# givemeone1astkiss/RNA-MPNN

Measured on AMD Instinct MI355X. Metric: nucleotides/sec (forward), k=30 RNA graphs, higher is better.
Workload: dtype bf16; 1 GPU; C2: batch=256 RNAs, n~U[100,140], k=30, default 10-layer RNAMPNN, P=T; max_len=140, weights=closed-form deterministic init (3,536,900 params), parallelism=dp1

## Files before the change

rna-mpnn_amd/csrc/api.cpp:

```cpp
#include "api_internal.h"
#include "kernels_bf16.h"

#include <cstdarg>
#include <cstdlib>
#include <cstdio>
#include <cstring>
#include <string>
#include <vector>

static thread_local char g_err[512] = "";

int fail(int code, const char* fmt, ...) {
    va_list ap;
    va_start(ap, fmt);
    vsnprintf(g_err, sizeof(g_err), fmt, ap);
    va_end(ap);
    return code;
}

extern "C" const char* rnampnn_last_error(void) { return g_err; }
extern "C" const char* rnampnn_version(void) { return "rnampnn-hip 0.1 (gfx950)"; }

static int add_raw(rnampnn_ctx* c, const std::string& key, int64_t numel) {
    RawT t{key, numel, c->raw_floats, false};
// ... 459 lines not shown
}

static void run_ffn(Run& r, const Chain& ch, const std::vector<Lin>& ffn, const float* x, int ldx, float* out) {
    if (run_chain(r, ch, ffn, x, ldx, nullptr, 0, out, ffn.back().out)) return;
    const float* cur = x;
    int ld = ldx;
    float* bufs[2] = {r.w.s0, r.w.s1};
    for (size_t i = 0; i < ffn.size(); ++i) {
        bool last = i + 1 == ffn.size();
        float* dst = last ? out : bufs[i & 1];
        gemm(r, ffn[i], cur, ld, dst, ffn[i].out);
        cur = dst; ld = ffn[i].out;
    }
}

static NodeJob node_job(rnampnn_ctx* c, const Mlp2& m, bf16_t* p, bf16_t* q) {
    NodeJob j;
    j.img = derp<bf16_t>(c, m.pq_img); j.bias = derp<float>(c, m.pq_bp); j.p = p; j.q = q; j.p_efrag = m.depth == 1;
    return j;
}
static void node_pq(Run& r, const Mlp2& m, const float* h, bool edge) {
    rnampnn_ctx* c = r.c;
    if (r.fast)
        launch_node_update(r.pk, h, nullptr, nullptr, 0, nullptr, nullptr, 1,
                           node_job(c, m, edge ? r.w.p_e : r.w.p_m, edge ? r.w.q_e : r.w.q_m), NodeJob{}, r.s);
    else
        launch_gemm_f32(r.ntot(), r.pk.Nmax, h, RN_D, RN_D, nullptr, 0, 0, derp<float>(c, m.pq_t),
                        derp<float>(c, m.pq_b), 256, 0, nullptr, 0, edge ? r.w.pq_e : r.w.pq_m, 256, r.s);
}

static MpnnW32 w32(rnampnn_ctx* c, const Mlp2& m) {
    MpnnW32 w;
    w.wc_t = derp<float>(c, m.wc_t);
    w.w2_t = m.depth > 1 ? derp<float>(c, m.w2_t) : nullptr;
    w.b2 = m.depth > 1 ? rawp(c, m.b[1]) : nullptr;
    w.depth = m.depth;
    return w;
}
static MpnnWB wbf(rnampnn_ctx* c, const Mlp2& m) {
    MpnnWB w;
    w.img = derp<bf16_t>(c, m.img);
    w.b2p = derp<float>(c, m.b2p);
    return w;
}

static void mpnn_step(Run& r, const Mlp2* we, const Mlp2* wm, const float* h_in, float* h_pre, float* msg_out, bool embed_first = false,
                      int reverse = 0) {
    rnampnn_ctx* c = r.c;
    int k = c->cfg.num_res_neighbours;
    bool timed = c->prof && c->ev_used + 2 <= c->ev.size() && (c->prof_seen++ % c->prof_stride) == 0;
    if (timed) { c->ev_kind[c->ev_used / 2] = (we && wm) ? 0 : 1; (void)hipEventRecord(c->ev[c->ev_used], r.s); }
    if (embed_first) {
        launch_resmpnn_embed_bf16(r.pk, k, r.w.nbr, (bf16_t*)r.w.e, r.w.geomh, derp<bf16_t>(c, c->edge_embed_img), rawp(c, c->edge_embed[0].b),
                                  derp<float>(c, c->edge_embed_b1p), r.w.p_m, r.w.q_m, wbf(c, *wm), h_pre, h_in, reverse, r.s);
    } else if (r.fast) {
        launch_mpnn_bf16(r.pk, k, we != nullptr, wm != nullptr, r.w.nbr, (bf16_t*)r.w.e, r.w.p_e, r.w.q_e, r.w.p_m,
                         r.w.q_m, we ? wbf(c, *we) : MpnnWB{}, wm ? wbf(c, *wm) : MpnnWB{}, h_pre, msg_out, we && we->depth == 1,
                         wm ? h_in : nullptr, reverse, r.s);
    } else {
        MpnnW32 e32 = we ? w32(c, *we) : MpnnW32{}, m32 = wm ? w32(c, *wm) : MpnnW32{};
        launch_mpnn_f32(r.pk, k, we != nullptr, wm != nullptr, r.w.nbr, (float*)r.w.e, r.w.pq_e, r.w.pq_m, e32, m32,
                        h_in, h_pre, msg_out, r.s);
    }
    if (timed) { (void)hipEventRecord(c->ev[c->ev_used + 1], r.s); c->ev_used += 2; }
}

static void unpack_e(Run& r, float* dst) {
    int k = r.c->cfg.num_res_neighbours;
    if (r.fast) {
        launch_efrag_to_rows((const bf16_t*)r.w.e, r.ntot(), r.pk.Nmax, k, r.w.big, r.s);
        launch_unpack_edges(r.pk, k, r.w.big, r.w.nbr, dst, r.s);
    } else {
        launch_unpack_edges(r.pk, k, (const float*)r.w.e, r.w.nbr, dst, r.s);
    }
}

static int begin_run(Run& r, rnampnn_handle h, const float* mask, int B, int T, void* ws, size_t ws_bytes, void* stream,
                     const int32_t* cu_seqlens = nullptr, int n_total = 0) {
    if (!h) return fail(RNAMPNN_ERR_BAD_ARG, "null handle");
    if (!h->finalized) return fail(RNAMPNN_ERR_WEIGHTS, "weights not finalized (call rnampnn_finalize_weights)");
    if ((!mask && !cu_seqlens) || !ws || B <= 0 || T <= 0) return fail(RNAMPNN_ERR_BAD_ARG, "null pointer or non-positive B/T");
    const long long nmax = cu_seqlens ? (long long)n_total : (long long)B * T;
    if (nmax <= 0 || nmax > 0x3fffffffLL / (h->cfg.num_res_neighbours * 4))
        return fail(RNAMPNN_ERR_BAD_ARG, "row count out of range for 32-bit edge indexing; split the batch");
    size_t need = carve(h, B, (size_t)nmax, nullptr, nullptr);
    if (ws_bytes < need) return fail(RNAMPNN_ERR_WORKSPACE, "workspace %zu bytes < required %zu", ws_bytes, need);
    if (((uintptr_t)ws & 255) != 0) return fail(RNAMPNN_ERR_BAD_ARG, "workspace must be 256-byte aligned");
    r.c = h;
    r.s = (hipStream_t)stream;
    r.fast = h->cfg.precision == RNAMPNN_PREC_BF16;
    carve(h, B, (size_t)nmax, (char*)ws, &r.w);
    r.pk.len = r.w.len; r.pk.cu = r.w.cu; r.pk.node_b = r.w.node_b;
    r.pk.B = B; r.pk.T = T; r.pk.Nmax = (int)nmax; r.pk.packed_in = cu_seqlens ? 1 : 0;
    size_t Nmax = r.pk.Nmax;
    ZeroRegions z{};
    auto add = [&](void* p, size_t bytes) { z.ptr[z.n] = p; z.words[z.n] = (unsigned)(bytes / 4); ++z.n; };
    add(r.w.hA + Nmax * RN_D, RN_D * sizeof(float));
    add(r.w.hB + Nmax * RN_D, RN_D * sizeof(float));
    if (r.fast) {
        add(r.w.p_e + Nmax * RN_D, RN_D * sizeof(bf16_t));
        add(r.w.p_m + Nmax * RN_D, RN_D * sizeof(bf16_t));
        add(r.w.q_e + Nmax * RN_D, RN_D * sizeof(bf16_t));
        add(r.w.q_m + Nmax * RN_D, RN_D * sizeof(bf16_t));
    } else {
        add(r.w.pq_e + Nmax * 256, 256 * sizeof(float));
        add(r.w.pq_m + Nmax * 256, 256 * sizeof(float));
    }
    if (cu_seqlens) launch_lengths_from_cu(cu_seqlens, r.pk, r.s);
    else launch_lengths(mask, r.pk, r.s);
    launch_zero_regions(z, r.s);
    return RNAMPNN_OK;
}

struct PackedOut { float* logits; float* embedding; int n_total; };
static int forward_core(Run& r, rnampnn_handle h, const RnaMpnnForwardIO* io, const PackedOut* po);

extern "C" int rnampnn_forward(rnampnn_handle h, const RnaMpnnForwardIO* io, void* ws, size_t ws_bytes, void* stream) {
    if (!io || !io->coords) return fail(RNAMPNN_ERR_BAD_ARG, "rnampnn_forward: null io/coords");
    if (io->stop_after == 0 && !io->logits && !io->embedding)
        return fail(RNAMPNN_ERR_BAD_ARG, "rnampnn_forward: logits (or embedding) output required");
    Run r;
    int rc = begin_run(r, h, io->mask, io->B, io->T, ws, ws_bytes, stream);
    if (rc) return rc;
    return forward_core(r, h, io, nullptr);
}

extern "C" int rnampnn_forward_packed(rnampnn_handle h, const float* coords_packed, const int32_t* cu_seqlens, int32_t B,
                                      int32_t N_total, int32_t T_max, int32_t T_norm, float* logits_packed,
                                      float* embedding_packed, void* ws, size_t ws_bytes, void* stream) {
    if (!coords_packed || !cu_seqlens || (!logits_packed && !embedding_packed))
        return fail(RNAMPNN_ERR_BAD_ARG, "rnampnn_forward_packed: null input or no output");
    Run r;
    int rc = begin_run(r, h, nullptr, B, T_max, ws, ws_bytes, stream, cu_seqlens, N_total);
    if (rc) return rc;
    RnaMpnnForwardIO io;
    memset(&io, 0, sizeof(io));
    io.coords = coords_packed; io.B = B; io.T = T_max; io.T_norm = T_norm;
    PackedOut po{logits_packed, embedding_packed, N_total};
    return forward_core(r, h, &io, &po);
}

static int forward_core(Run& r, rnampnn_handle h, const RnaMpnnForwardIO* io, const PackedOut* po) {
    int rc = RNAMPNN_OK;
    rnampnn_ctx* c = h;
    const RnaMpnnConfig& g = c->cfg;
    if (io->T > g.padding_len)
        return fail(RNAMPNN_ERR_T_GT_P, "max_len %d exceeds padding_len %d", io->T, g.padding_len);
    int k = g.num_res_neighbours, L = g.num_res_mpnn_layers;
    int t_norm = io->T_norm > 0 ? io->T_norm : io->T;
    if (t_norm < io->T) return fail(RNAMPNN_ERR_BAD_ARG, "T_norm %d < T %d", t_norm, io->T);
    Ws& w = r.w;
    hipStream_t s = r.s;

    launch_geom(io->coords, r.pk, t_norm, io->raw, w.raw_p, w.geom, r.fast ? w.geomh : nullptr, s);
    const bool fused_first = r.fast && io->stop_after != 1;
    {
        const Lin& l = c->raw_project;
        launch_gemm_f32(r.ntot(), r.pk.Nmax, w.raw_p, RN_RAWP, l.in_pad, nullptr, 0, 0, derp<float>(c, l.wt), rawp(c, l.b), l.out,
                        l.gelu ? 1 : 0, nullptr, 0, w.n0, RN_D, r.s);
    }
    rc = run_bert(r, c->emb, w.n0, w.n1);
    if (!rc) {
        if (fused_first)
            launch_node_update(r.pk, w.n1, rawp(c, c->feat_gn_scale), rawp(c, c->feat_gn_shift), t_norm, w.coef, w.hA, 1,
                               node_job(c, c->mpnn[0].msg, w.p_m, w.q_m), NodeJob{}, r.s);
        else
            launch_graph_norm_packed(r.pk, w.n1, w.hA, rawp(c, c->feat_gn_scale), rawp(c, c->feat_gn_shift), t_norm, r.s);
    }
    if (rc) return rc;
    if (launch_knn(io->coords, r.pk, t_norm, k, w.nbr, io->edge_index, s))
        return fail(RNAMPNN_ERR_UNSUPPORTED, "max_len %d too long for the LDS-resident k-NN row", io->T);
    const bool embed_first = fused_first && L >= 1 && !io->e0 && resmpnn_covers(k, false, false) && !ab_switch("RNAMPNN_EMBED_TWO_LAUNCH");
    if (embed_first) { }
    else if (r.fast)
        launch_edge_embed_bf16(r.pk, k, w.geomh, w.nbr, derp<bf16_t>(c, c->edge_embed_img), rawp(c, c->edge_embed[0].b),
                               derp<float>(c, c->edge_embed_b1p), (bf16_t*)w.e, s);
    else
        launch_edge_embed_f32(r.pk, k, w.geom, w.nbr, derp<float>(c, c->edge_embed[0].wt), rawp(c, c->edge_embed[0].b),
                              g.depth_res_edge_feature > 1 ? derp<float>(c, c->edge_embed[1].wt) : nullptr,
                              g.depth_res_edge_feature > 1 ? rawp(c, c->edge_embed[1].b) : nullptr,
                              g.depth_res_edge_feature, (float*)w.e, s);
    if (io->h0) launch_unpack_nodes(r.pk, w.hA, RN_D, RN_D, io->h0, s);
    if (io->e0) unpack_e(r, io->e0);
    if (io->stop_after == 1) { HIP_TRY(hipGetLastError()); return RNAMPNN_OK; }

    if (!fused_first) node_pq(r, c->mpnn[0].msg, w.hA, false);
    bool edge_pending = false;
    int n_fused = 0;
    for (int l = 0; l < L; ++l) {
        mpnn_step(r, edge_pending ? &c->mpnn[l - 1].edge : nullptr, &c->mpnn[l].msg, w.hA, w.hB, nullptr, l == 0 && embed_first, n_fused++ & 1);
        bool tap_e = io->tap_layer == l + 1 && io->e_layer;
        edge_pending = l + 1 < L;
        const bool need_e = edge_pending || tap_e, need_m = l + 1 < L;
        const float* gsc = rawp(c, c->mpnn[l].gn_scale);
        const float* gsh = rawp(c, c->mpnn[l].gn_shift);
        if (r.fast && (need_e || need_m)) {
            const NodeJob je = need_e ? node_job(c, c->mpnn[l].edge, w.p_e, w.q_e) : NodeJob{};
            const NodeJob jm = need_m ? node_job(c, c->mpnn[l + 1].msg, w.p_m, w.q_m) : NodeJob{};
            launch_node_update(r.pk, w.hB, gsc, gsh, t_norm, w.coef, w.hA, (need_e && need_m) ? 2 : 1, need_e ? je : jm, jm, s);
        } else {
            launch_graph_norm_packed(r.pk, w.hB, w.hA, gsc, gsh, t_norm, s);
            if (need_e) node_pq(r, c->mpnn[l].edge, w.hA, true);
            if (need_m) node_pq(r, c->mpnn[l + 1].msg, w.hA, false);
        }
        if (io->tap_layer == l + 1) {
            if (io->h_layer) launch_unpack_nodes(r.pk, w.hA, RN_D, RN_D, io->h_layer, s);
            if (tap_e) {
                mpnn_step(r, &c->mpnn[l].edge, nullptr, w.hA, w.hB, nullptr, false, n_fused++ & 1);
                edge_pending = false;
                unpack_e(r, io->e_layer);
            }
        }
    }
    float* raw_emb = w.n2;
    rc = run_bert(r, c->post, w.hA, w.n0);
    if (rc) return rc;
    run_ffn(r, c->raw_chain, c->raw_ffn, w.raw_p, RN_RAWP, w.n1);
    launch_graph_norm_packed(r.pk, w.n1, w.n2, rawp(c, c->rawffn_gn_scale), rawp(c, c->rawffn_gn_shift), t_norm, s);
    if (io->h_post) launch_unpack_nodes(r.pk, w.n0, RN_D, RN_D, io->h_post, s);
    if (io->raw_emb) launch_unpack_nodes(r.pk, raw_emb, RN_D, RN_D, io->raw_emb, s);
    if (io->embedding) {
        launch_unpack_nodes_strided(r.pk, w.n0, RN_D, RN_D, io->embedding, 2 * RN_D, 0, s);
        launch_unpack_nodes_strided(r.pk, raw_emb, RN_D, RN_D, io->embedding, 2 * RN_D, RN_D, s);
    }
    if (po && po->embedding) {
        HIP_TRY(hipMemcpy2DAsync(po->embedding, 2 * RN_D * sizeof(float), w.n0, RN_D * sizeof(float), RN_D * sizeof(float),
                                 po->n_total, hipMemcpyDeviceToDevice, s));
        HIP_TRY(hipMemcpy2DAsync(po->embedding + RN_D, 2 * RN_D * sizeof(float), raw_emb, RN_D * sizeof(float),
                                 RN_D * sizeof(float), po->n_total, hipMemcpyDeviceToDevice, s));
    }
    const bool want_logits = io->logits || (po && po->logits);
    float* logits_rows = (po && po->logits) ? po->logits : w.logits_p;
    if (want_logits && run_chain(r, c->readout_chain, c->readout, w.n0, RN_D, raw_emb, RN_D, logits_rows, 4)) {
        if (io->logits) launch_unpack_nodes(r.pk, logits_rows, 4, 4, io->logits, s);
    } else if (want_logits) {
        const float* cur = nullptr;
        int ld = 0;
        float* bufs[2] = {w.s0, w.s1};
        for (size_t i = 0; i < c->readout.size(); ++i) {
            const Lin& l = c->readout[i];
            bool last = i + 1 == c->readout.size();
            float* dst = last ? logits_rows : bufs[i & 1];
            if (i == 0) gemm(r, l, w.n0, RN_D, dst, l.out, nullptr, 0, raw_emb, RN_D, RN_D);
            else gemm(r, l, cur, ld, dst, l.out);
            cur = dst; ld = l.out;
        }
        if (io->logits) launch_unpack_nodes(r.pk, logits_rows, 4, 4, io->logits, s);
    }
    HIP_TRY(hipGetLastError());
    return RNAMPNN_OK;
}

extern "C" int rnampnn_mpnn_layer(rnampnn_handle h, int32_t layer, const float* h_in, const float* e_in,
                                  const int64_t* edge_index, const float* mask, int32_t B, int32_t T, int32_t T_norm,
                                  float* msg_out, float* h_out, float* e_out, void* ws, size_t ws_bytes, void* stream) {
    if (!h_in || !e_in || !edge_index) return fail(RNAMPNN_ERR_BAD_ARG, "rnampnn_mpnn_layer: null input");
    Run r;
    int rc = begin_run(r, h, mask, B, T, ws, ws_bytes, stream);
    if (rc) return rc;
    rnampnn_ctx* c = h;
    if (layer < 0 || layer >= c->cfg.num_res_mpnn_layers) return fail(RNAMPNN_ERR_BAD_ARG, "layer %d out of range", layer);
    int k = c->cfg.num_res_neighbours;
    int t_norm = T_norm > 0 ? T_norm : T;
    Ws& w = r.w;
    hipStream_t s = r.s;
    launch_pack_nodes(r.pk, h_in, RN_D, w.hA, RN_D, s);
    launch_pack_index(r.pk, k, edge_index, w.nbr, s);
    if (r.fast) {
        launch_pack_edges(r.pk, k, e_in, w.big, s);
        launch_rows_to_efrag(w.big, r.ntot(), r.pk.Nmax, k, w.nbr, (bf16_t*)w.e, s);
    } else {
        launch_pack_edges(r.pk, k, e_in, (float*)w.e, s);
    }
    const MpnnLayer& m = c->mpnn[layer];
    node_pq(r, m.msg, w.hA, false);
    float* msg_p = msg_out ? w.big : nullptr;
    mpnn_step(r, nullptr, &m.msg, w.hA, w.hB, msg_p);
    if (msg_out) launch_unpack_edges(r.pk, k, w.big, nullptr, msg_out, s);
    if (h_out || e_out) {
        launch_graph_norm_packed(r.pk, w.hB, w.hA, rawp(c, m.gn_scale), rawp(c, m.gn_shift), t_norm, s);
        if (h_out) launch_unpack_nodes(r.pk, w.hA, RN_D, RN_D, h_out, s);
        if (e_out) {
            node_pq(r, m.edge, w.hA, true);
            mpnn_step(r, &m.edge, nullptr, w.hA, w.hB, nullptr);
            unpack_e(r, e_out);
        }
    }
    HIP_TRY(hipGetLastError());
    return RNAMPNN_OK;
}

extern "C" int rnampnn_graph_norm(const float* x, const float* mask, const float* scale, const float* shift,
                                  int32_t B, int32_t T, int32_t T_tot, int32_t D, float* y, void* stream) {
    if (!x || !mask || !scale || !shift || !y || B <= 0 || T <= 0 || D <= 0)
        return fail(RNAMPNN_ERR_BAD_ARG, "rnampnn_graph_norm: bad argument");
    if (T_tot <= 0) T_tot = T;
    if (T_tot < T) return fail(RNAMPNN_ERR_BAD_ARG, "T_tot %d < T %d", T_tot, T);
    launch_graph_norm_padded(x, mask, scale, shift, B, T, T_tot, D, y, (hipStream_t)stream);
    HIP_TRY(hipGetLastError());
    return RNAMPNN_OK;
}

extern "C" int rnampnn_rnabert(rnampnn_handle h, int32_t which, const float* x, const float* mask, int32_t B, int32_t T,
                               float* y, void* ws, size_t ws_bytes, void* stream) {
    if (!x || !y) return fail(RNAMPNN_ERR_BAD_ARG, "rnampnn_rnabert: null tensor");
    Run r;
    int rc = begin_run(r, h, mask, B, T, ws, ws_bytes, stream);
// ... 77 lines not shown
```

rna-mpnn_amd/csrc/kernels_f32.hip:

```cpp
#include "api_internal.h"
#include "bf16_core.h"
#include "graph_norm_dev.h"
#include <cstdlib>

#define WAVE 64
static constexpr float kLEPS = 1.0e6f;

__device__ __forceinline__ float wave_sum(float v) {
#pragma unroll
    for (int o = 32; o > 0; o >>= 1) v += __shfl_xor(v, o, WAVE);
    return v;
}

__global__ void k_lengths(const float* __restrict__ mask, int B, int T, int* __restrict__ len) {
    int b = blockIdx.x;
    float s = 0.f;
    for (int t = threadIdx.x; t < T; t += WAVE) s += mask[(size_t)b * T + t];
    s = wave_sum(s);
    if (threadIdx.x == 0) len[b] = (int)(s + 0.5f);
}

__device__ __forceinline__ int block_exclusive_scan_1024(int v, int* wave_tot , int* total) {
    const int lane = threadIdx.x & 63, wave = threadIdx.x >> 6;
    int inc = v;
// ... 22 lines not shown

__global__ void __launch_bounds__(1024) k_lengths_from_cu(const int32_t* __restrict__ cu_in, int B, int T, int Nmax,
                                                          int* __restrict__ len, int* __restrict__ cu) {
    __shared__ int wave_tot[16];
    const int tid = threadIdx.x;
    const int chunk = (B + 1023) / 1024;
    const int lo = min(B, tid * chunk), hi = min(B, lo + chunk);
    int s = 0;
    for (int i = lo; i < hi; ++i) s += min(max(cu_in[i + 1] - cu_in[i], 0), T);
    int total;
    int run = block_exclusive_scan_1024(s, wave_tot, &total);
    if (tid == 0) cu[B] = min(total, Nmax);
    for (int i = lo; i < hi; ++i) {
        const int l = min(max(cu_in[i + 1] - cu_in[i], 0), T);
        const int c0 = min(run, Nmax);
        cu[i] = c0;
        len[i] = min(l, Nmax - c0);
        run += l;
    }
}
__global__ void k_zero_regions(ZeroRegions z) {
    const int g = blockIdx.x;
    if (g >= z.n) return;
    unsigned* p = reinterpret_cast<unsigned*>(z.ptr[g]);
    for (unsigned i = threadIdx.x; i < z.words[g]; i += blockDim.x) p[i] = 0u;
}
__global__ void k_zero_bytes(uint4* __restrict__ p, size_t n16, unsigned char* __restrict__ tail, int ntail) {
    const uint4 z = make_uint4(0u, 0u, 0u, 0u);
    for (size_t i = (size_t)blockIdx.x * blockDim.x + threadIdx.x; i < n16; i += (size_t)gridDim.x * blockDim.x) p[i] = z;
    if (blockIdx.x == 0 && (int)threadIdx.x < ntail) tail[threadIdx.x] = 0;
}
void launch_zero_bytes(void* ptr, size_t bytes, hipStream_t s) {
    if (!bytes) return;
    const size_t n16 = bytes / 16;
    size_t g = (n16 + 255) / 256;
    if (g > 2048) g = 2048;
    if (g < 1) g = 1;
    hipLaunchKernelGGL(k_zero_bytes, dim3((unsigned)g), dim3(256), 0, s, reinterpret_cast<uint4*>(ptr), n16,
                       reinterpret_cast<unsigned char*>(ptr) + n16 * 16, (int)(bytes - n16 * 16));
}
__global__ void k_copy16(const uint4* __restrict__ src, uint4* __restrict__ dst, size_t n16) {
    for (size_t i = (size_t)blockIdx.x * blockDim.x + threadIdx.x; i < n16; i += (size_t)gridDim.x * blockDim.x) dst[i] = src[i];
}
void launch_copy_bytes(void* dst, const void* src, size_t bytes, hipStream_t s) {
    const size_t n16 = bytes / 16;
    if (!n16) return;
    size_t g = (n16 + 255) / 256;
    if (g > 2048) g = 2048;
    hipLaunchKernelGGL(k_copy16, dim3((unsigned)g), dim3(256), 0, s, reinterpret_cast<const uint4*>(src), reinterpret_cast<uint4*>(dst), n16);
}
void launch_zero_regions(const ZeroRegions& z, hipStream_t s) {
    if (z.n > 0) hipLaunchKernelGGL(k_zero_regions, dim3(z.n), dim3(256), 0, s, z);
}

void launch_lengths_from_cu(const int32_t* cu_seqlens, const PackInfo& pk, hipStream_t s) {
    hipLaunchKernelGGL(k_lengths_from_cu, dim3(1), dim3(1024), 0, s, cu_seqlens, pk.B, pk.T, pk.Nmax, pk.len, pk.cu);
}

void launch_lengths(const float* mask, const PackInfo& pk, hipStream_t s) {
    hipLaunchKernelGGL(k_lengths, dim3(pk.B), dim3(WAVE), 0, s, mask, pk.B, pk.T, pk.len);
    hipLaunchKernelGGL(k_scan, dim3(1), dim3(1024), 0, s, pk.len, pk.B, pk.cu);
}

__device__ __forceinline__ void geom_record(const float* c, float* g) {
#pragma unroll
    for (int i = 0; i < 21; ++i) g[i] = c[i];
    float v[5][3];
#pragma unroll
    for (int a = 0; a < 5; ++a) {
#pragma unroll
        for (int d = 0; d < 3; ++d) v[a][d] = c[(a + 1) * 3 + d] - c[a * 3 + d];
        float nr = sqrtf(v[a][0] * v[a][0] + v[a][1] * v[a][1] + v[a][2] * v[a][2]);
        float inv = 1.0f / fmaxf(nr, 1e-12f);
#pragma unroll
        for (int d = 0; d < 3; ++d) g[21 + a * 3 + d] = v[a][d] * inv;
    }
#pragma unroll
    for (int a = 0; a < 4; ++a) {
        float x = v[a][1] * v[a + 1][2] - v[a][2] * v[a + 1][1];
        float y = v[a][2] * v[a + 1][0] - v[a][0] * v[a + 1][2];
        float z = v[a][0] * v[a + 1][1] - v[a][1] * v[a + 1][0];
        float inv = 1.0f / fmaxf(sqrtf(x * x + y * y + z * z), kSEPS);
        g[36 + a * 3 + 0] = x * inv; g[36 + a * 3 + 1] = y * inv; g[36 + a * 3 + 2] = z * inv;
    }
}

__device__ __forceinline__ void geomh_record(const float* g, float* gh) {
#pragma unroll
    for (int i = 0; i < RN_GEOMH; ++i) gh[i] = 0.f;
#pragma unroll
    for (int h = 0; h < 2; ++h) {
#pragma unroll
        for (int a = 0; a < 4; ++a)
            if (4 * h + a < 7)
#pragma unroll
                for (int d = 0; d < 3; ++d) gh[32 * h + 3 * a + d] = g[(4 * h + a) * 3 + d];
#pragma unroll
        for (int a = 0; a < 3; ++a)
            if (3 * h + a < 5)
#pragma unroll
                for (int d = 0; d < 3; ++d) gh[32 * h + 12 + 3 * a + d] = g[21 + (3 * h + a) * 3 + d];
#pragma unroll
        for (int a = 0; a < 2; ++a)
#pragma unroll
            for (int d = 0; d < 3; ++d) gh[32 * h + 21 + 3 * a + d] = g[36 + (2 * h + a) * 3 + d];
    }
}

__device__ __forceinline__ void raw_features(const float* c, float* f) {
    int o = 0;
#pragma unroll
    for (int a = 0; a < 7; ++a)
#pragma unroll
        for (int b = a + 1; b < 7; ++b) {
            float dx = c[a * 3] - c[b * 3], dy = c[a * 3 + 1] - c[b * 3 + 1], dz = c[a * 3 + 2] - c[b * 3 + 2];
            f[o++] = sqrtf(dx * dx + dy * dy + dz * dz + kSEPS);
        }
    float v[5][3], nr[5], u[5][3];
#pragma unroll
    for (int a = 0; a < 5; ++a) {
#pragma unroll
        for (int d = 0; d < 3; ++d) v[a][d] = c[(a + 1) * 3 + d] - c[a * 3 + d];
        nr[a] = sqrtf(v[a][0] * v[a][0] + v[a][1] * v[a][1] + v[a][2] * v[a][2]);
        float inv = 1.0f / fmaxf(nr[a], kSEPS);
#pragma unroll
        for (int d = 0; d < 3; ++d) u[a][d] = v[a][d] * inv;
    }
#pragma unroll
    for (int a = 0; a < 4; ++a)
        f[21 + a] = (v[a][0] * v[a + 1][0] + v[a][1] * v[a + 1][1] + v[a][2] * v[a + 1][2]) / (nr[a] * nr[a + 1] + kSEPS);
    float nm[4][3];
#pragma unroll
    for (int a = 0; a < 4; ++a) {
        float x = u[a][1] * u[a + 1][2] - u[a][2] * u[a + 1][1];
        float y = u[a][2] * u[a + 1][0] - u[a][0] * u[a + 1][2];
        float z = u[a][0] * u[a + 1][1] - u[a][1] * u[a + 1][0];
        float inv = 1.0f / fmaxf(sqrtf(x * x + y * y + z * z), kSEPS);
        nm[a][0] = x * inv; nm[a][1] = y * inv; nm[a][2] = z * inv;
    }
#pragma unroll
    for (int a = 0; a < 3; ++a) f[25 + a] = nm[a + 1][0] * nm[a][0] + nm[a + 1][1] * nm[a][1] + nm[a + 1][2] * nm[a][2];
}

__device__ __forceinline__ void store_geomh(const float* g, float* __restrict__ dst) {
    float gh[RN_GEOMH];
    geomh_record(g, gh);
#pragma unroll
    for (int i = 0; i < RN_GEOMH; i += 4) *reinterpret_cast<float4*>(dst + i) = make_float4(gh[i], gh[i + 1], gh[i + 2], gh[i + 3]);
}

__device__ __forceinline__ void store_geom(const float* c, float* __restrict__ geom, float* __restrict__ geomh, size_t row) {
    float g[RN_GEOM];
    geom_record(c, g);
    float* gp = geom + row * RN_GEOM;
#pragma unroll
    for (int i = 0; i < RN_GEOM; ++i) gp[i] = g[i];
    if (geomh) store_geomh(g, geomh + row * RN_GEOMH);
}

__global__ void k_geom(const float* __restrict__ coords, PackInfo pk, int Tp, float* __restrict__ raw_out,
                       float* __restrict__ raw_p, float* __restrict__ geom, float* __restrict__ geomh) {
    int id = blockIdx.x * blockDim.x + threadIdx.x;
    if (id >= pk.B * pk.T) {
        const int b = id - pk.B * pk.T;
        if (b < pk.B && pk.len[b] == pk.T && pk.T < Tp) {
            float c[21];
#pragma unroll
            for (int i = 0; i < 21; ++i) c[i] = 0.f;
            store_geom(c, geom, geomh, (size_t)(pk.Nmax + b));
        }
        return;
    }
    int b = id / pk.T, t = id - b * pk.T;
    int n = pk.len[b];
    float c[21];
    const bool have = !pk.packed_in || t < n;
    const float* src = coords + (size_t)(pk.packed_in ? pk.cu[b] + (t < n ? t : 0) : id) * 21;
#pragma unroll
    for (int i = 0; i < 21; ++i) c[i] = have ? src[i] : 0.f;
    if (t < n) {
        int p = pk.cu[b] + t;
        pk.node_b[p] = b;
        float f[28];
        raw_features(c, f);
        float* rp = raw_p + (size_t)p * RN_RAWP;
#pragma unroll
        for (int i = 0; i < 28; ++i) rp[i] = f[i];
#pragma unroll
        for (int i = 28; i < RN_RAWP; ++i) rp[i] = 0.f;
        if (raw_out) {
            float* ro = raw_out + (size_t)id * RN_RAW;
#pragma unroll
            for (int i = 0; i < 28; ++i) ro[i] = f[i];
        }
        store_geom(c, geom, geomh, (size_t)p);
    } else {
        if (raw_out) {
            float* ro = raw_out + (size_t)id * RN_RAW;
#pragma unroll
            for (int i = 0; i < 21; ++i) ro[i] = kLEPS;
#pragma unroll
            for (int i = 21; i < 28; ++i) ro[i] = 0.f;
        }
        if (t == n) store_geom(c, geom, geomh, (size_t)(pk.Nmax + b));
    }
}

void launch_geom(const float* coords, const PackInfo& pk, int Tp, float* raw_out, float* raw_p, float* geom, float* geomh, hipStream_t s) {
    int total = pk.B * (pk.T + 1);
    hipLaunchKernelGGL(k_geom, dim3((total + 63) / 64), dim3(64), 0, s, coords, pk, Tp, raw_out, raw_p, geom, geomh);
}

template <int G>
__global__ void __launch_bounds__(256) k_knn(const float* __restrict__ coords, PackInfo pk, int Tp, int k, int rows_per_block,
                                              int* __restrict__ nbr, int64_t* __restrict__ eidx) {
    extern __shared__ __attribute__((aligned(16))) float sm[];
    constexpr int GROUPS = 256 / G;
    int b = blockIdx.x;
    int n = pk.len[b];
    int T = pk.T;
    int row0 = blockIdx.y * rows_per_block;
    if (row0 >= T) return;
    int gl = threadIdx.x % G, grp = threadIdx.x / G;
    float* cen = sm;
    float* drow = sm + 3 * T + grp * T;
    if (row0 < n) {
        for (int j = threadIdx.x; j < n; j += 256) {
            const float* c = coords + (size_t)(pk.packed_in ? pk.cu[b] + j : b * T + j) * 21;
            float sx = 0.f, sy = 0.f, sz = 0.f;
#pragma unroll
            for (int a = 0; a < 7; ++a) { sx += c[a * 3]; sy += c[a * 3 + 1]; sz += c[a * 3 + 2]; }
            cen[j * 3] = sx / 7.0f; cen[j * 3 + 1] = sy / 7.0f; cen[j * 3 + 2] = sz / 7.0f;
        }
    }
    __syncthreads();
    int base = pk.cu[b];
    const int row_end = min(T, row0 + rows_per_block);
    for (int i0 = row0; i0 < row_end; i0 += GROUPS) {
        const int i = i0 + grp;
        const bool row_live = i < row_end;
        const bool real = row_live && i < n;
        if (row_live && !real) {
            if (eidx) for (int s = gl; s < k; s += G) eidx[((size_t)b * T + i) * k + s] = -1;
        }
        float cx = 0.f, cy = 0.f, cz = 0.f;
        if (real) { cx = cen[i * 3]; cy = cen[i * 3 + 1]; cz = cen[i * 3 + 2]; }
        if (real) {
            for (int j = gl; j < n; j += G) {
                float dx = __fsub_rn(cen[j * 3], cx), dy = __fsub_rn(cen[j * 3 + 1], cy), dz = __fsub_rn(cen[j * 3 + 2], cz);
                float ss = __fadd_rn(__fadd_rn(__fmul_rn(dx, dx), __fmul_rn(dy, dy)), __fmul_rn(dz, dz));
                drow[j] = (j == i) ? 3.0e38f : sqrtf(__fadd_rn(ss, kSEPS));
            }
        }
        const int nreal = real ? min(k, n - 1) : 0;
        int nmax = nreal;
#pragma unroll
        for (int o = G; o < 64; o <<= 1) nmax = max(nmax, __shfl_xor(nmax, o, 64));
        unsigned long long prev = 0ull;
        const size_t pbase = (size_t)(base + i) * k;
        const size_t obase = ((size_t)b * T + i) * k;
        if constexpr (G == 64) {
            auto wave_min = [](unsigned long long v) {
#pragma unroll
                for (int o = 32; o > 0; o >>= 1) { const unsigned long long other = __shfl_xor(v, o, 64); v = other < v ? other : v; }
                return v;
            };
            unsigned long long cand = ~0ull;
            if (real)
                for (int j = gl; j < n; j += 64) {
                    const unsigned long long key = ((unsigned long long)__float_as_uint(drow[j]) << 32) | (unsigned)j;
                    cand = key < cand ? key : cand;
                }
            for (int s = 0; s < nreal; ++s) {
                const unsigned long long best = wave_min(cand);
                const int jw = (int)(best & 0xffffffffu), w = jw & 63;
                if (gl == 0) {
                    nbr[pbase + s] = base + jw;
                    if (eidx) eidx[obase + s] = jw;
                }
                unsigned long long nc = ~0ull;
                for (int j = w + 64 * gl; j < n; j += 64 * 64) {
                    const unsigned long long key = ((unsigned long long)__float_as_uint(drow[j]) << 32) | (unsigned)j;
                    if (key > best && key < nc) nc = key;
                }
                nc = wave_min(nc);
                if (gl == w) cand = nc;
            }
        } else {
        for (int s = 0; s < nmax; ++s) {
            unsigned long long best = ~0ull;
            if (s < nreal) {
                for (int j = gl; j < n; j += G) {
                    unsigned long long key = ((unsigned long long)__float_as_uint(drow[j]) << 32) | (unsigned)j;
                    if (key > prev && key < best) best = key;
                }
            }
#pragma unroll
            for (int o = G / 2; o > 0; o >>= 1) {
                unsigned long long other = __shfl_xor(best, o, 64);
                best = other < best ? other : best;
            }
            prev = best;
            if (gl == 0 && s < nreal) {
                int j = (int)(best & 0xffffffffu);
                nbr[pbase + s] = base + j;
                if (eidx) eidx[obase + s] = j;
            }
        }
        }
        if (real) {
            for (int s = nreal + gl; s < k; s += G) {
                bool phantom = (s == n - 1) && (n < Tp);
                nbr[pbase + s] = phantom ? pk.Nmax + b : -1;
                if (eidx) eidx[obase + s] = phantom ? n : -1;
            }
        }
    }
}

template <int NK>
__global__ void __launch_bounds__(256) k_knn_queue(const float* __restrict__ coords, PackInfo pk, int Tp, int k, int rows_per_block,
                                                    int* __restrict__ nbr, int64_t* __restrict__ eidx) {
    extern __shared__ __attribute__((aligned(16))) float sm[];
    constexpr int G = 16, GROUPS = 256 / G;
    const int b = blockIdx.x;
    const int n = pk.len[b];
    const int T = pk.T;
    const int row0 = blockIdx.y * rows_per_block;
    if (row0 >= T) return;
    const int gl = threadIdx.x % G, grp = threadIdx.x / G;
    float* cen = sm;
    if (row0 < n) {
        for (int j = threadIdx.x; j < n; j += 256) {
            const float* c = coords + (size_t)(pk.packed_in ? pk.cu[b] + j : b * T + j) * 21;
            float sx = 0.f, sy = 0.f, sz = 0.f;
#pragma unroll
            for (int a = 0; a < 7; ++a) { sx += c[a * 3]; sy += c[a * 3 + 1]; sz += c[a * 3 + 2]; }
            cen[j * 3] = sx / 7.0f; cen[j * 3 + 1] = sy / 7.0f; cen[j * 3 + 2] = sz / 7.0f;
        }
    }
    __syncthreads();
    const int base = pk.cu[b];
    const int row_end = min(T, row0 + rows_per_block);
    for (int i0 = row0; i0 < row_end; i0 += GROUPS) {
        const int i = i0 + grp;
        const bool row_live = i < row_end;
        const bool real = row_live && i < n;
        if (row_live && !real) {
            if (eidx) for (int s = gl; s < k; s += G) eidx[((size_t)b * T + i) * k + s] = -1;
        }
        float cx = 0.f, cy = 0.f, cz = 0.f;
        if (real) { cx = cen[i * 3]; cy = cen[i * 3 + 1]; cz = cen[i * 3 + 2]; }
        unsigned long long q[NK];
#pragma unroll
        for (int t = 0; t < NK; ++t) {
            const int j = gl + G * t;
            unsigned long long key = ~0ull;
            if (real && j < n && j != i) {
                float dx = __fsub_rn(cen[j * 3], cx), dy = __fsub_rn(cen[j * 3 + 1], cy), dz = __fsub_rn(cen[j * 3 + 2], cz);
                float ss = __fadd_rn(__fadd_rn(__fmul_rn(dx, dx), __fmul_rn(dy, dy)), __fmul_rn(dz, dz));
                key = ((unsigned long long)__float_as_uint(sqrtf(__fadd_rn(ss, kSEPS))) << 32) | (unsigned)j;
            }
            q[t] = key;
        }
#pragma unroll
        for (int pass = 0; pass < NK; ++pass)
#pragma unroll
            for (int t = pass & 1; t + 1 < NK; t += 2) {
                const unsigned long long lo = q[t] < q[t + 1] ? q[t] : q[t + 1], hi = q[t] < q[t + 1] ? q[t + 1] : q[t];
                q[t] = lo; q[t + 1] = hi;
            }
        const int nreal = real ? min(k, n - 1) : 0;
        int nmax = nreal;
#pragma unroll
        for (int o = G; o < 64; o <<= 1) nmax = max(nmax, __shfl_xor(nmax, o, 64));
        const size_t pbase = (size_t)(base + i) * k;
        const size_t obase = ((size_t)b * T + i) * k;
        for (int s = 0; s < nmax; ++s) {
            unsigned long long best = q[0];
#define KNN_ROR(n) do {                                                                                                      \
                const unsigned lo_ = (unsigned)__builtin_amdgcn_update_dpp(0, (int)(unsigned)best, 0x120 + (n), 0xf, 0xf, false);            \
                const unsigned hi_ = (unsigned)__builtin_amdgcn_update_dpp(0, (int)(unsigned)(best >> 32), 0x120 + (n), 0xf, 0xf, false);     \
                const unsigned long long other_ = ((unsigned long long)hi_ << 32) | lo_;                                     \
                best = other_ < best ? other_ : best;                                                                        \
            } while (0)
            KNN_ROR(8); KNN_ROR(4); KNN_ROR(2); KNN_ROR(1);
#undef KNN_ROR
            if (q[0] == best && best != ~0ull) {
#pragma unroll
                for (int t = 0; t + 1 < NK; ++t) q[t] = q[t + 1];
                q[NK - 1] = ~0ull;
            }
            if (gl == 0 && s < nreal) {
                const int j = (int)(best & 0xffffffffu);
                nbr[pbase + s] = base + j;
                if (eidx) eidx[obase + s] = j;
            }
        }
        if (real) {
            for (int s = nreal + gl; s < k; s += G) {
                const bool phantom = (s == n - 1) && (n < Tp);
                nbr[pbase + s] = phantom ? pk.Nmax + b : -1;
                if (eidx) eidx[obase + s] = phantom ? n : -1;
            }
        }
    }
}

int launch_knn(const float* coords, const PackInfo& pk, int Tp, int k, int* nbr, int64_t* eidx, hipStream_t s) {
    if (pk.T <= 256) {
        const int rpb = 32;
        dim3 grid(pk.B, (pk.T + rpb - 1) / rpb);
        const size_t lds = (size_t)3 * pk.T * sizeof(float);
        if (pk.T <= 64) hipLaunchKernelGGL(k_knn_queue<4>, grid, dim3(256), lds, s, coords, pk, Tp, k, rpb, nbr, eidx);
        else if (pk.T <= 144) hipLaunchKernelGGL(k_knn_queue<9>, grid, dim3(256), lds, s, coords, pk, Tp, k, rpb, nbr, eidx);
        else hipLaunchKernelGGL(k_knn_queue<16>, grid, dim3(256), lds, s, coords, pk, Tp, k, rpb, nbr, eidx);
        return 0;
    }
    const size_t lds16 = (size_t)(3 + 16) * pk.T * sizeof(float);
    if (lds16 <= 48 * 1024) {
        int rpb = 32;
        dim3 grid(pk.B, (pk.T + rpb - 1) / rpb);
        hipLaunchKernelGGL(k_knn<16>, grid, dim3(256), lds16, s, coords, pk, Tp, k, rpb, nbr, eidx);
        return 0;
    }
    size_t lds = (size_t)(3 + 4) * pk.T * sizeof(float);
    if (lds > 160 * 1024 - 256) return 1;
    static DevAttr attr;
    ensure_dyn_lds((const void*)k_knn<64>, lds, attr);
    int rpb = pk.T <= 512 ? 16 : 64;
    dim3 grid(pk.B, (pk.T + rpb - 1) / rpb);
    hipLaunchKernelGGL(k_knn<64>, grid, dim3(256), lds, s, coords, pk, Tp, k, rpb, nbr, eidx);
    return 0;
}

__device__ __forceinline__ void tile_fma(const float* __restrict__ Xs, int ldx, int K, const float* __restrict__ Wt,
                                         int ldw, int c, int g, float (&acc)[16]) {
    const float* xr = Xs + g * 16 * ldx;
    for (int kk = 0; kk < K; kk += 4) {
        float w0 = Wt[(size_t)(kk + 0) * ldw + c], w1 = Wt[(size_t)(kk + 1) * ldw + c];
        float w2 = Wt[(size_t)(kk + 2) * ldw + c], w3 = Wt[(size_t)(kk + 3) * ldw + c];
#pragma unroll
        for (int r = 0; r < 16; ++r) {
            const float4 x = *reinterpret_cast<const float4*>(xr + r * ldx + kk);
            acc[r] = fmaf(x.x, w0, acc[r]); acc[r] = fmaf(x.y, w1, acc[r]);
            acc[r] = fmaf(x.z, w2, acc[r]); acc[r] = fmaf(x.w, w3, acc[r]);
        }
    }
}

#define EX_LD 100
#define EH_LD 132
__global__ void __launch_bounds__(256) k_edge_embed_f32(PackInfo pk, int k, const float* __restrict__ geom,
        const int* __restrict__ nbr, const float* __restrict__ w0t, const float* __restrict__ b0,
        const float* __restrict__ w1t, const float* __restrict__ b1, int depth, float* __restrict__ e) {
    __shared__ __attribute__((aligned(16))) float X[32 * EX_LD];
    __shared__ __attribute__((aligned(16))) float H[32 * EH_LD];
    __shared__ int valid_s[32];
    int ntot = pk.cu[pk.B];
    for (int p = blockIdx.x; p < ntot; p += gridDim.x) {
        int tid = threadIdx.x;
        if (tid < 32) {
            int j = (tid < k) ? nbr[(size_t)p * k + tid] : -1;
            valid_s[tid] = j >= 0;
            float* x = X + tid * EX_LD;
            if (j >= 0) {
                const float* gi = geom + (size_t)p * RN_GEOM;
                const float* gj = geom + (size_t)j * RN_GEOM;
                float cj[RN_GEOM];
#pragma unroll
                for (int i = 0; i < RN_GEOM; ++i) cj[i] = gj[i];
#pragma unroll
                for (int a = 0; a < 7; ++a) {
                    float ax = gi[a * 3], ay = gi[a * 3 + 1], az = gi[a * 3 + 2];
#pragma unroll
                    for (int bb = 0; bb < 7; ++bb) {
                        float dx = ax - cj[bb * 3], dy = ay - cj[bb * 3 + 1], dz = az - cj[bb * 3 + 2];
                        x[a * 7 + bb] = sqrtf(dx * dx + dy * dy + dz * dz + kSEPS);
                    }
                }
#pragma unroll
                for (int a = 0; a < 5; ++a) {
                    float ax = gi[21 + a * 3], ay = gi[22 + a * 3], az = gi[23 + a * 3];
#pragma unroll
                    for (int bb = 0; bb < 5; ++bb)
                        x[49 + a * 5 + bb] = ax * cj[21 + bb * 3] + ay * cj[22 + bb * 3] + az * cj[23 + bb * 3];
                }
#pragma unroll
                for (int a = 0; a < 4; ++a) {
                    float ax = gi[36 + a * 3], ay = gi[37 + a * 3], az = gi[38 + a * 3];
#pragma unroll
                    for (int bb = 0; bb < 4; ++bb)
                        x[74 + a * 4 + bb] = ax * cj[36 + bb * 3] + ay * cj[37 + bb * 3] + az * cj[38 + bb * 3];
                }
#pragma unroll
                for (int i = RN_ERAW; i < RN_ERAWP; ++i) x[i] = 0.f;
            } else {
                for (int i = 0; i < RN_ERAWP; ++i) x[i] = 0.f;
            }
        }
        __syncthreads();
        int c = tid & 127, g = tid >> 7;
        float acc[16];
        float bias = b0[c];
#pragma unroll
        for (int r = 0; r < 16; ++r) acc[r] = bias;
        tile_fma(X, EX_LD, RN_ERAWP, w0t, RN_D, c, g, acc);
#pragma unroll
        for (int r = 0; r < 16; ++r) acc[r] = gelu_erf(acc[r]);
        if (depth > 1) {
#pragma unroll
            for (int r = 0; r < 16; ++r) H[(g * 16 + r) * EH_LD + c] = acc[r];
            __syncthreads();
            bias = b1[c];
#pragma unroll
            for (int r = 0; r < 16; ++r) acc[r] = bias;
            tile_fma(H, EH_LD, RN_D, w1t, RN_D, c, g, acc);
#pragma unroll
            for (int r = 0; r < 16; ++r) acc[r] = gelu_erf(acc[r]);
        }
#pragma unroll
        for (int r = 0; r < 16; ++r) {
            int s = g * 16 + r;
            if (s < k) e[((size_t)p * k + s) * RN_D + c] = valid_s[s] ? acc[r] : 0.f;
        }
        __syncthreads();
    }
}

void launch_edge_embed_f32(const PackInfo& pk, int k, const float* geom, const int* nbr, const float* w0t,
                           const float* b0, const float* w1t, const float* b1, int depth, float* e, hipStream_t s) {
    int grid = pk.Nmax < 4096 ? pk.Nmax : 4096;
    hipLaunchKernelGGL(k_edge_embed_f32, dim3(grid), dim3(256), 0, s, pk, k, geom, nbr, w0t, b0, w1t, b1, depth, e);
}

template <bool DO_EDGE, bool DO_MSG>
__global__ void __launch_bounds__(256) k_mpnn_f32(PackInfo pk, int k, const int* __restrict__ nbr, float* __restrict__ e,
        const float* __restrict__ pq_e, const float* __restrict__ pq_m, MpnnW32 we, MpnnW32 wm,
        const float* __restrict__ h_in, float* __restrict__ h_pre, float* __restrict__ msg_out) {
    __shared__ __attribute__((aligned(16))) float X[32 * EH_LD];
    __shared__ __attribute__((aligned(16))) float H[32 * EH_LD];
    __shared__ int jrow[32];
    __shared__ float part[128];
    int ntot = pk.cu[pk.B];
    int tid = threadIdx.x, c = tid & 127, g = tid >> 7;
    for (int p = blockIdx.x; p < ntot; p += gridDim.x) {
        if (tid < 32) jrow[tid] = (tid < k) ? nbr[(size_t)p * k + tid] : -1;
        for (int idx = tid; idx < 32 * 32; idx += 256) {
            int r = idx >> 5, q = idx & 31;
            float4 v = make_float4(0.f, 0.f, 0.f, 0.f);
            if (r < k) v = *reinterpret_cast<const float4*>(e + ((size_t)p * k + r) * RN_D + q * 4);
            *reinterpret_cast<float4*>(X + r * EH_LD + q * 4) = v;
        }
        __syncthreads();
        float acc[16];
        if (DO_EDGE) {
            float pi = pq_e[(size_t)p * 256 + c];
#pragma unroll
            for (int r = 0; r < 16; ++r) {
                int j = jrow[g * 16 + r];
                j = j < 0 ? 0 : (j > pk.Nmax ? pk.Nmax : j);
                acc[r] = pi + pq_e[(size_t)j * 256 + 128 + c];
            }
            tile_fma(X, EH_LD, RN_D, we.wc_t, RN_D, c, g, acc);
#pragma unroll
            for (int r = 0; r < 16; ++r) acc[r] = gelu_erf(acc[r]);
            if (we.depth > 1) {
#pragma unroll
                for (int r = 0; r < 16; ++r) H[(g * 16 + r) * EH_LD + c] = acc[r];
// ... 428 lines not shown
```

Baseline: 14.20 million nucleotides/s.

## Rework k-NN queue merge with LDS-spilled queues and 32-bit DPP reductions

The per-lane sorted candidate queue in the k-NN kernel is now spilled to LDS after sorting, keeping only the head in registers. Each merge step uses two 32-bit row-of-16 DPP min reductions (distance, then index) instead of 64-bit key reductions, and results are gathered into one lane per slot so writes are coalesced across the 16-lane group. The loop bound is made wave-uniform without shuffles. Separately, the fp32 geometry buffer is no longer written when the fast path only consumes the packed geomh buffer. The trade-offs are extra LDS per block and the assumption that nothing on the fast path reads w.geom.

```diff
diff --git a/rna-mpnn_amd/csrc/api.cpp b/rna-mpnn_amd/csrc/api.cpp
--- a/rna-mpnn_amd/csrc/api.cpp
+++ b/rna-mpnn_amd/csrc/api.cpp
@@ -635,7 +635,7 @@
     Ws& w = r.w;
     hipStream_t s = r.s;
 
-    launch_geom(io->coords, r.pk, t_norm, io->raw, w.raw_p, w.geom, r.fast ? w.geomh : nullptr, s);
+    launch_geom(io->coords, r.pk, t_norm, io->raw, w.raw_p, r.fast ? nullptr : w.geom, r.fast ? w.geomh : nullptr, s);
     const bool fused_first = r.fast && io->stop_after != 1;
     {
         const Lin& l = c->raw_project;
diff --git a/rna-mpnn_amd/csrc/kernels_f32.hip b/rna-mpnn_amd/csrc/kernels_f32.hip
--- a/rna-mpnn_amd/csrc/kernels_f32.hip
+++ b/rna-mpnn_amd/csrc/kernels_f32.hip
@@ -198,9 +198,11 @@
 __device__ __forceinline__ void store_geom(const float* c, float* __restrict__ geom, float* __restrict__ geomh, size_t row) {
     float g[RN_GEOM];
     geom_record(c, g);
-    float* gp = geom + row * RN_GEOM;
-#pragma unroll
-    for (int i = 0; i < RN_GEOM; ++i) gp[i] = g[i];
+    if (geom) {
+        float* gp = geom + row * RN_GEOM;
+#pragma unroll
+        for (int i = 0; i < RN_GEOM; ++i) gp[i] = g[i];
+    }
     if (geomh) store_geomh(g, geomh + row * RN_GEOMH);
 }
 
@@ -364,18 +366,27 @@
     }
 }
 
+template <int NK> constexpr int knn_queue_lds_bytes(int T) { return ((3 * T + 3) & ~3) * 4 + NK * 256 * 8; }
+
+__device__ __forceinline__ unsigned row16_min_u32(unsigned v) {
+#define KNN_ROR(n) v = min(v, (unsigned)__builtin_amdgcn_update_dpp(0, (int)v, 0x120 + (n), 0xf, 0xf, false))
+    KNN_ROR(8); KNN_ROR(4); KNN_ROR(2); KNN_ROR(1);
+#undef KNN_ROR
+    return v;
+}
+
 template <int NK>
-__global__ void __launch_bounds__(256) k_knn_queue(const float* __restrict__ coords, PackInfo pk, int Tp, int k, int rows_per_block,
-                                                    int* __restrict__ nbr, int64_t* __restrict__ eidx) {
-    extern __shared__ __attribute__((aligned(16))) float sm[];
+__device__ __forceinline__ void knn_queue_role(const float* __restrict__ coords, const PackInfo& pk, int Tp, int k, int rows_per_block,
+                                               const int b, const int rowblk, int* __restrict__ nbr, int64_t* __restrict__ eidx, float* sm) {
     constexpr int G = 16, GROUPS = 256 / G;
-    const int b = blockIdx.x;
     const int n = pk.len[b];
     const int T = pk.T;
-    const int row0 = blockIdx.y * rows_per_block;
+    const int row0 = rowblk * rows_per_block;
     if (row0 >= T) return;
     const int gl = threadIdx.x % G, grp = threadIdx.x / G;
     float* cen = sm;
+    uint2* const qb = reinterpret_cast<uint2*>(sm + ((3 * T + 3) & ~3)) + threadIdx.x;
+    qb[(NK - 1) * 256] = make_uint2(~0u, ~0u);
     if (row0 < n) {
         for (int j = threadIdx.x; j < n; j += 256) {
             const float* c = coords + (size_t)(pk.packed_in ? pk.cu[b] + j : b * T + j) * 21;
@@ -388,6 +399,7 @@
     __syncthreads();
     const int base = pk.cu[b];
     const int row_end = min(T, row0 + rows_per_block);
+    const int wave_row = __builtin_amdgcn_readfirstlane((int)threadIdx.x >> 6) * (64 / G);
     for (int i0 = row0; i0 < row_end; i0 += GROUPS) {
         const int i = i0 + grp;
         const bool row_live = i < row_end;
@@ -416,51 +428,54 @@
                 const unsigned long long lo = q[t] < q[t + 1] ? q[t] : q[t + 1], hi = q[t] < q[t + 1] ? q[t + 1] : q[t];
                 q[t] = lo; q[t + 1] = hi;
             }
+#pragma unroll
+        for (int t = 1; t < NK; ++t) qb[(t - 1) * 256] = make_uint2((unsigned)(q[t] >> 32), (unsigned)q[t]);
+        unsigned hd = (unsigned)(q[0] >> 32), hj = (unsigned)q[0];
+        int hs = 0;
         const int nreal = real ? min(k, n - 1) : 0;
-        int nmax = nreal;
-#pragma unroll
-        for (int o = G; o < 64; o <<= 1) nmax = max(nmax, __shfl_xor(nmax, o, 64));
+        const int nmax = i0 + wave_row < min(row_end, n) ? min(k, n - 1) : 0;
         const size_t pbase = (size_t)(base + i) * k;
         const size_t obase = ((size_t)b * T + i) * k;
-        for (int s = 0; s < nmax; ++s) {
-            unsigned long long best = q[0];
-#define KNN_ROR(n) do {                                                                                                      \
-                const unsigned lo_ = (unsigned)__builtin_amdgcn_update_dpp(0, (int)(unsigned)best, 0x120 + (n), 0xf, 0xf, false);            \
-                const unsigned hi_ = (unsigned)__builtin_amdgcn_update_dpp(0, (int)(unsigned)(best >> 32), 0x120 + (n), 0xf, 0xf, false);     \
-                const unsigned long long other_ = ((unsigned long long)hi_ << 32) | lo_;                                     \
-                best = other_ < best ? other_ : best;                                                                        \
-            } while (0)
-            KNN_ROR(8); KNN_ROR(4); KNN_ROR(2); KNN_ROR(1);
-#undef KNN_ROR
-            if (q[0] == best && best != ~0ull) {
-#pragma unroll
-                for (int t = 0; t + 1 < NK; ++t) q[t] = q[t + 1];
-                q[NK - 1] = ~0ull;
-            }
-            if (gl == 0 && s < nreal) {
-                const int j = (int)(best & 0xffffffffu);
-                nbr[pbase + s] = base + j;
-                if (eidx) eidx[obase + s] = j;
-            }
-        }
-        if (real) {
-            for (int s = nreal + gl; s < k; s += G) {
-                const bool phantom = (s == n - 1) && (n < Tp);
-                nbr[pbase + s] = phantom ? pk.Nmax + b : -1;
-                if (eidx) eidx[obase + s] = phantom ? n : -1;
-            }
-        }
-    }
-}
+        for (int s0 = 0; s0 < k; s0 += G) {
+            unsigned res = 0u;
+            for (int u = 0; u < G; ++u) {
+                if (s0 + u >= nmax) break;
+                const unsigned dmin = row16_min_u32(hd);
+                const unsigned cj = hd == dmin ? hj : ~0u;
+                const unsigned jmin = row16_min_u32(cj);
+                if (cj == jmin && jmin != ~0u) {
+                    const uint2 h = qb[hs];
+                    hs += 256;
+                    hd = h.x; hj = h.y;
+                }
+                res = gl == u ? jmin : res;
+            }
+            const int s = s0 + gl;
+            if (real && s < k) {
+                const bool found = s < nreal, phantom = (s == n - 1) && (n < Tp);
+                nbr[pbase + s] = found ? base + (int)res : phantom ? pk.Nmax + b : -1;
+                if (eidx) eidx[obase + s] = found ? (int)res : phantom ? n : -1;
+            }
+        }
+    }
+}
+
+template <int NK>
+__global__ void __launch_bounds__(256) k_knn_queue(const float* __restrict__ coords, PackInfo pk, int Tp, int k, int rows_per_block,
+                                                    int* __restrict__ nbr, int64_t* __restrict__ eidx) {
+    extern __shared__ __attribute__((aligned(16))) float sm[];
+    knn_queue_role<NK>(coords, pk, Tp, k, rows_per_block, blockIdx.x, blockIdx.y, nbr, eidx, sm);
+}
+
+static constexpr int kKnnQueueRows = 32;
 
 int launch_knn(const float* coords, const PackInfo& pk, int Tp, int k, int* nbr, int64_t* eidx, hipStream_t s) {
     if (pk.T <= 256) {
-        const int rpb = 32;
+        const int rpb = kKnnQueueRows;
         dim3 grid(pk.B, (pk.T + rpb - 1) / rpb);
-        const size_t lds = (size_t)3 * pk.T * sizeof(float);
-        if (pk.T <= 64) hipLaunchKernelGGL(k_knn_queue<4>, grid, dim3(256), lds, s, coords, pk, Tp, k, rpb, nbr, eidx);
-        else if (pk.T <= 144) hipLaunchKernelGGL(k_knn_queue<9>, grid, dim3(256), lds, s, coords, pk, Tp, k, rpb, nbr, eidx);
-        else hipLaunchKernelGGL(k_knn_queue<16>, grid, dim3(256), lds, s, coords, pk, Tp, k, rpb, nbr, eidx);
+        if (pk.T <= 64) hipLaunchKernelGGL(k_knn_queue<4>, grid, dim3(256), knn_queue_lds_bytes<4>(pk.T), s, coords, pk, Tp, k, rpb, nbr, eidx);
+        else if (pk.T <= 144) hipLaunchKernelGGL(k_knn_queue<9>, grid, dim3(256), knn_queue_lds_bytes<9>(pk.T), s, coords, pk, Tp, k, rpb, nbr, eidx);
+        else hipLaunchKernelGGL(k_knn_queue<16>, grid, dim3(256), knn_queue_lds_bytes<16>(pk.T), s, coords, pk, Tp, k, rpb, nbr, eidx);
         return 0;
     }
     const size_t lds16 = (size_t)(3 + 16) * pk.T * sizeof(float);
```

Measured after the change: 14.35 million nucleotides/s (median of 6 runs). 1.01x the previous value.
